# thetumbled/pulsar-tlaplus

Measured on AMD Instinct MI355X. Metric: distinct states/sec, compaction.tla scaled cfg, 1/2/4/8 MI355X vs host TLC, higher is better.
Workload: dtype u64

## Files before the change

include/tlcgpu.h:

```cpp
#ifndef TLCGPU_H
#define TLCGPU_H
#include <stdint.h>

#ifdef __cplusplus
extern "C" {
#endif

#define TLCG_ABI_VERSION 4
#define TLCG_MAX_SET 63
#define TLCG_MAX_INV 8

enum {
  TLCG_INV_TYPESAFE = 0,
  TLCG_INV_COMPACTED_LEDGER_LEAK = 1,
  TLCG_INV_HORIZON_CORRECTNESS = 2,
  TLCG_INV_DUP_NULLKEY_MESSAGE = 3,
  TLCG_INV_USER = 16
};

enum {
  TLCG_ACT_INIT = -1,
  TLCG_ACT_PRODUCER = 0,
  TLCG_ACT_PHASE_ONE,
  TLCG_ACT_PHASE_TWO_WRITE,
// ... 35 lines not shown
typedef struct tlcg_opts {
  int32_t device;
  int32_t log2_fpset_slots;
  uint64_t state_capacity;
  int32_t tlc_order;
  int32_t rank, world;
  int32_t partition;
  int32_t engine;
  int32_t spill;
  uint64_t device_store_cap;
  int32_t fpset_spill;
  int32_t log2_fpset_max;
  int32_t outdegree;
  int32_t reserved[1];
} tlcg_opts;

enum { TLCG_ENGINE_AUTO = 0, TLCG_ENGINE_GLOBAL = 1, TLCG_ENGINE_COMPONENT = 2,
       TLCG_ENGINE_TREE = 3  };

typedef struct tlcg_stats {
  uint64_t generated;
  uint64_t distinct;
  uint64_t frontier;
  int32_t depth;
  int32_t status;
  int32_t invariant;
  int32_t action;
  uint64_t event_gidx;
  double fp_collision_optimistic;
  double kernel_ms;
  double expand_ms;
  uint64_t levels_redone;
  uint64_t engine;
  uint64_t jit_used;
  uint64_t host_states;
  uint64_t fpset_host_states;
  uint64_t transport;
  uint64_t tlc_exact;
} tlcg_stats;

typedef struct tlcg_ctx tlcg_ctx;

int tlcg_abi_version(void);
int tlcg_check_model(const tlcg_model* m, char* err, int32_t cap);
int tlcg_state_bits(const tlcg_model* m);
int tlcg_state_words(const tlcg_model* m);
uint64_t tlcg_init_count(const tlcg_model* m);

int tlcg_create(const tlcg_model* m, const tlcg_opts* o, tlcg_ctx** out);
void tlcg_destroy(tlcg_ctx* c);
const char* tlcg_last_error(const tlcg_ctx* c);

int tlcg_init(tlcg_ctx* c, tlcg_stats* st);
int tlcg_step_level(tlcg_ctx* c, tlcg_stats* st);
int tlcg_run(tlcg_ctx* c, tlcg_stats* st);

int tlcg_level_sizes(tlcg_ctx* c, uint64_t* out, int32_t cap, int32_t* n);
int tlcg_trace(tlcg_ctx* c, uint64_t* states, int32_t* actions, int32_t cap, int32_t* len);
int tlcg_state_at(tlcg_ctx* c, uint64_t gidx, uint64_t* state, uint64_t* parent_ref);
int tlcg_copy_states(tlcg_ctx* c, uint64_t first, uint64_t n, uint64_t* out);
int tlcg_trace_words(tlcg_ctx* c, uint64_t* states, int32_t* actions, int32_t cap, int32_t* len);
int tlcg_state_at_words(tlcg_ctx* c, uint64_t gidx, uint64_t* state, uint64_t* parent_ref);
int tlcg_copy_states_words(tlcg_ctx* c, uint64_t first, uint64_t n, uint64_t* out);
int tlcg_tlc_stop_stats(tlcg_ctx* c, uint64_t* generated, uint64_t* distinct, uint64_t* left_on_queue);
int tlcg_outdegree(tlcg_ctx* c, uint64_t* hist, int32_t cap, int32_t* n);
int tlcg_expansions(tlcg_ctx* c, uint64_t* out);
int tlcg_level_generated(tlcg_ctx* c, uint64_t* out, int32_t cap, int32_t* n);
int tlcg_ordinal_bits(const tlcg_model* m);
int tlcg_action_of_ordinal(const tlcg_model* m, int32_t ordinal);

int tlcg_decode(const tlcg_model* m, uint64_t state, char* buf, int32_t cap);
uint64_t tlcg_host_init_state(const tlcg_model* m, uint64_t idx);
int tlcg_host_successors(const tlcg_model* m, uint64_t state, uint64_t* out, int32_t* actions, int32_t cap);
int tlcg_host_check_invariants(const tlcg_model* m, uint64_t state);
int tlcg_decode_words(const tlcg_model* m, const uint64_t* state, char* buf, int32_t cap);
int tlcg_host_init_state_words(const tlcg_model* m, uint64_t idx, uint64_t* out);
int tlcg_host_successors_words(const tlcg_model* m, const uint64_t* state, uint64_t* out, int32_t* actions,
                               int32_t cap);
int tlcg_host_check_invariants_words(const tlcg_model* m, const uint64_t* state);
int tlcg_host_check_invariants_batch(const tlcg_model* m, const uint64_t* states, uint64_t n, int32_t* out);
int64_t tlcg_host_component_selfcheck(const tlcg_model* m, uint64_t first, uint64_t n);
int64_t tlcg_host_lane_inv_selfcheck(const tlcg_model* m);
int64_t tlcg_host_lane_owner_selfcheck(const tlcg_model* m, int* overflow);
int64_t tlcg_host_lane_owner_word(const tlcg_model* m, uint32_t code);
int tlcg_host_tree_slot_probes(const tlcg_model* m, uint64_t comp, int64_t* out);
int64_t tlcg_host_termination_counterexample(const tlcg_model* m);
enum { TLCG_FAIR_NONE = 0, TLCG_FAIR_WF_NEXT = 1 };
enum { TLCG_LIVE_HOLDS = 0, TLCG_LIVE_STUTTERING = 1, TLCG_LIVE_CYCLE = 2 };
typedef struct tlcg_liveness {
  int32_t holds;
  int32_t kind;
  int32_t fairness;
  int32_t depth;
  uint64_t states_notp;
  uint64_t init_notp;
  uint64_t edges_notp;
  uint64_t stuck;
  uint64_t on_cycles;
  uint64_t peel_rounds;
  int32_t trace_len;
  int32_t loop_to;
  int32_t back_action;
  int32_t reserved;
  double kernel_ms;
  double wall_ms;
} tlcg_liveness;
int tlcg_check_termination(const tlcg_model* m, const tlcg_opts* o, int32_t fairness, tlcg_liveness* out,
                           uint64_t* states, int32_t* actions, int32_t cap, int32_t* len, char* err,
                           int32_t err_cap);
int tlcg_liveness_graph_selftest(const uint32_t* row, const uint32_t* col, const uint8_t* is_p, uint32_t n,
                                 uint32_t n_init, int32_t words, const tlcg_opts* o, int32_t fairness,
                                 tlcg_liveness* out, uint64_t* states, int32_t* actions, int32_t cap, int32_t* len,
                                 char* err, int32_t err_cap);

enum { TLCG_PROP_EVENTUALLY = 0, TLCG_PROP_INFINITELY_OFTEN = 1, TLCG_PROP_LEADS_TO = 2 };
typedef struct tlcg_property {
  tlcg_liveness lv;
  int32_t form;
  int32_t seed_at;
  uint64_t reachable;
  uint64_t seeds;
  int64_t error_state;
  double classify_ms;
} tlcg_property;
int tlcg_check_property(const tlcg_model* m, const tlcg_opts* o, int32_t fairness, const char* name,
                        tlcg_property* out, uint64_t* states, int32_t* actions, int32_t cap, int32_t* len,
                        char* err, int32_t err_cap);
int tlcg_property_graph_selftest(const uint32_t* row, const uint32_t* col, const uint8_t* is_p, const uint8_t* is_q,
                                 uint32_t n, uint32_t n_init, int32_t words, const tlcg_opts* o, int32_t fairness,
                                 int32_t form, tlcg_property* out, uint64_t* states, int32_t* actions, int32_t cap,
                                 int32_t* len, char* err, int32_t err_cap);
int tlcg_host_property_form(const tlcg_model* m, const char* name, int32_t* form, char* err, int32_t cap);
int tlcg_host_property_eval(const tlcg_model* m, const char* name, const uint64_t* states, uint64_t n, uint8_t* out);

typedef struct tlcg_action_property {
  int32_t holds;
  int32_t depth;
  uint64_t reachable;
  uint64_t steps;
  uint64_t violating;
  uint64_t erroring;
  int32_t step_depth;
  int32_t step_action;
  int32_t trace_len;
  int32_t reserved;
  int64_t error_state;
  double kernel_ms;
  double check_ms;
  double wall_ms;
} tlcg_action_property;
int tlcg_check_action_property(const tlcg_model* m, const tlcg_opts* o, const char* name, tlcg_action_property* out,
                               uint64_t* states, int32_t* actions, int32_t cap, int32_t* len, char* err,
                               int32_t err_cap);
int tlcg_action_property_graph_selftest(const uint32_t* row, const uint32_t* col, const uint8_t* verdict, uint32_t n,
                                        uint32_t n_init, int32_t words, const tlcg_opts* o,
                                        tlcg_action_property* out, uint64_t* states, int32_t* actions, int32_t cap,
                                        int32_t* len, char* err, int32_t err_cap);
int tlcg_host_action_property_form(const tlcg_model* m, const char* name, uint32_t* var_mask, char* err, int32_t cap);
int tlcg_host_action_property_eval(const tlcg_model* m, const char* name, const uint64_t* pairs, uint64_t n,
                                   uint8_t* out);
int tlcg_action_eval_selftest(const tlcg_model* m, const tlcg_opts* o, const char* name, const uint64_t* pairs,
                              uint64_t n, uint8_t* out, char* err, int32_t cap);

int tlcg_peer_access(int32_t n);
int tlcg_device_count(void);
int tlcg_owner(tlcg_ctx* c, uint64_t state);
// ... 44 lines not shown
```

pulsar-tlaplus_amd/csrc/component_lane.h:

```cpp
#pragma once
#if !defined(__HIPCC_RTC__)
#include "component_body.h"
#endif

namespace tlcg {

#ifndef TLCG_LANE_R
#define TLCG_LANE_R 16
#endif
constexpr int LANE_R = TLCG_LANE_R;
#ifndef TLCG_LANE_STEP_TAB
#define TLCG_LANE_STEP_TAB 1
#endif
#ifndef TLCG_LANE_INV_FEAT
#define TLCG_LANE_INV_FEAT 1
#endif
#if defined(TLCG_USER_INV) || defined(TLCG_LANE_INV_UNCOND)
#undef TLCG_LANE_INV_FEAT
#define TLCG_LANE_INV_FEAT 0
#endif
#ifndef TLCG_LANE_OWNER_RING
#define TLCG_LANE_OWNER_RING 1
#endif
#if !TLCG_LANE_STEP_TAB
#undef TLCG_LANE_OWNER_RING
#define TLCG_LANE_OWNER_RING 0
#endif
#ifndef TLCG_LANE_FP_REG
#define TLCG_LANE_FP_REG 1
#endif
#ifndef TLCG_LANE_LEVEL_LDS
#define TLCG_LANE_LEVEL_LDS 1
#endif
#ifndef TLCG_LANE_CRASH_SKIP
#define TLCG_LANE_CRASH_SKIP 1
#endif

template <bool B>
struct lane_with2 {
  static constexpr bool value = B;
};

__device__ __forceinline__ uint32_t lane_wave_sum(uint32_t x) {
  x += (uint32_t)__builtin_amdgcn_update_dpp(0, (int)x, 0x111, 0xf, 0xf, true);
  x += (uint32_t)__builtin_amdgcn_update_dpp(0, (int)x, 0x112, 0xf, 0xf, true);
  x += (uint32_t)__builtin_amdgcn_update_dpp(0, (int)x, 0x114, 0xf, 0xf, true);
  x += (uint32_t)__builtin_amdgcn_update_dpp(0, (int)x, 0x118, 0xf, 0xf, true);
  return (uint32_t)__builtin_amdgcn_readlane((int)x, 15) + (uint32_t)__builtin_amdgcn_readlane((int)x, 31) +
         (uint32_t)__builtin_amdgcn_readlane((int)x, 47) + (uint32_t)__builtin_amdgcn_readlane((int)x, 63);
}

template <int K, bool OD = false>
__device__ __forceinline__ void component_lane_body(const CompArgs& a, const Layout& L) {
  static_assert(K <= 64, "records and the 16-bit level sums take K <= 64");
  static_assert(64 * (K - 2) * 4 < 65536, "level_add's 16-bit halves");
  constexpr int T = LANE_T, NW = T / 32, R = LANE_R;
  constexpr int LV = TLCG_CODE_MAXLV < COMP_MAXLV ? TLCG_CODE_MAXLV : COMP_MAXLV;
#if TLCG_LANE_OWNER_RING
  typedef uint32_t ring_t;
#else
  typedef uint16_t ring_t;
#endif
  __shared__ ring_t ring[R][64];
#if TLCG_LANE_FP_REG
  __shared__ u64 owner[T];
#else
  __shared__ uint32_t bits[NW][64];
  __shared__ uint32_t owner[T];
#endif
  constexpr int LVS = LV + (OD ? 3 : 0);
  static_assert(LVS <= 64 && (K - 2) * 4 + 1 < 256, "one lane per level sum; OD packs three counts above lgen's 8 bits");
  __shared__ unsigned long long lvl_sh[LVS];
#if TLCG_LANE_STEP_TAB
  __shared__ u64 steps[STEP_TAB];
#endif
  const int lane = threadIdx.x;
  const int mb = L.msg_sh + L.N * L.mw;
  const uint32_t mult = a.lane_mult;
#if TLCG_LANE_FP_REG
  for (int i = lane; i < T; i += 64) owner[i] = (u64)a.lane_owner[2 * i] | ((u64)a.lane_owner[2 * i + 1] << 32);
#else
  for (int i = lane; i < T; i += 64) owner[i] = a.lane_owner[2 * i];
#endif
#if TLCG_LANE_STEP_TAB
  for (int i = lane; i < STEP_TAB; i += 64) steps[i] = compactor_step_entry(L, i);
#endif
  if (lane < LVS) lvl_sh[lane] = 0;
  uint32_t gen = 0, dist = 0, nexp = 0;
  __syncthreads();
  auto level_add = [&](bool add, int lvc, uint32_t x) {
#if TLCG_LANE_LEVEL_LDS
    if (add) atomicAdd(&lvl_sh[lvc], (unsigned long long)(x & 0xFFFFu) | ((unsigned long long)(x >> 16) << 32));
#else
    const unsigned long long m = __ballot(add);
    if (!m) return;
    const int l0 = __builtin_amdgcn_readlane(lvc, __ffsll((long long)m) - 1);
    if (!__ballot(add && lvc != l0)) {
      const uint32_t s = lane_wave_sum(add ? x : 0u);
      if (lane == 0) atomicAdd(&lvl_sh[l0], (unsigned long long)(s & 0xFFFFu) | ((unsigned long long)(s >> 16) << 32));
    } else if (add) {
      atomicAdd(&lvl_sh[lvc], (unsigned long long)(x & 0xFFFFu) | ((unsigned long long)(x >> 16) << 32));
    }
#endif
  };
  for (u64 b = blockIdx.x; b * 64 < a.n_comp; b += gridDim.x) {
    const u64 ci = b * 64 + (u64)lane;
    const bool act = ci < a.n_comp;
    const u64 entry = act ? (a.list ? a.list[ci] : a.comp0 + ci) : 0;
    const u64 idx0 = entry & ((1ull << 40) - 1);
    const int counted = (int)(entry >> 40);
#if TLCG_LANE_FP_REG
    u64 fp = 0;
#else
#pragma unroll
    for (int i = 0; i < NW; ++i) bits[i][lane] = 0u;
#endif
    const u64 s0 = init_state(L, idx0);
    CodeConsts ccon = code_consts(L, comp_msgs_init(L, s0));
#ifdef TLCG_USER_INV
    code_consts_user(L, ccon);
#endif
#if TLCG_LANE_INV_FEAT
    const uint32_t cmask = lane_inv_mask(L, ccon);
#endif
#if TLCG_LANE_STEP_TAB
    const int term_c = lane_term_consts(L, ccon);
#endif
    const __amdgpu_buffer_rsrc_t rsrc = __builtin_amdgcn_make_buffer_rsrc(
        reinterpret_cast<uint32_t*>(a.store) + b * (u64)K * 64, (short)0, K * 64 * 4, 0x00020000);
    constexpr int OOB = 0x7fffffff;
    const unsigned loff = (unsigned)lane * 4u;
    int head = 0, tail = 0, level = 0, lvl_start = 0, lvl_end = 0;
    bool alive = act, ovf = false, stop = false;
    uint32_t lgen = 0, lvgen = 0;
    u64 lev = NO_EVENT;
    const lkey k0 = act ? (lkey)(s0 >> mb) : 0;
    const ckey c0 = code_encode(L, k0);
    const unsigned p0 = lane_slot(c0, mult);
    const uint32_t ow0 = (uint32_t)owner[p0];
    if (act && (code_decode(L, ccon, c0) != k0 || (ow0 & 0xFFFFu) != c0 + 1u)) {
      ovf = true;
      alive = false;
    }
    if (alive) {
#if TLCG_LANE_FP_REG
      fp = 1ull << (uint32_t)(owner[p0] >> 32);
#else
      bits[p0 >> 5][lane] = 1u << (p0 & 31);
#endif
#if TLCG_LANE_OWNER_RING
      ring[0][lane] = ow0;
#else
      ring[0][lane] = (uint16_t)c0;
#endif
      tail = 1;
      __builtin_amdgcn_raw_buffer_store_b32(comp_record(c0, 0, 0), rsrc, (int)loff, 0, 0);
      lgen = 1;
      const int c = check_invariants_direct(L, ccon, c0);
      if (c >= 0) {
        lev = make_comp_event(0, idx0, 0, 0, (c & 1) ? EVK_INV_ERROR : EVK_VIOLATION, c >> 1);
        alive = false;
        stop = true;
      }
    }
    lvl_end = tail;
#if TLCG_LANE_OWNER_RING
    uint32_t cur = ow0;
#else
    ckey cur = c0;
#endif
    while (__ballot(alive)) {
      const int tail0 = tail;
#if TLCG_LANE_OWNER_RING
      const ckey s = (cur & 0xFFFFu) - 1u;
      uint32_t nxt = 0, first_new = 0;
#else
      const ckey s = cur;
      ckey nxt = 0, first_new = 0;
#endif
      bool out = false, rare = false, dl = false, u1 = false, u2 = false;
      int q1 = INV_UNKNOWN + 1, q2 = INV_UNKNOWN + 1;
      ckey t = 0;
      int action = 0;
#if TLCG_LANE_OWNER_RING
      nxt = ring[(head + 1) & (R - 1)][lane];
      const uint32_t six = (cur >> LANE_OWNER_STEP_SH) & (uint32_t)(STEP_TAB - 1);
      uint32_t term = 0;
      const int r = compactor_step_ent(L, ccon, steps[six], six & 7u, s, &t, &action, &term);
#else
      nxt = ring[(head + 1) & (R - 1)][lane];
#if TLCG_LANE_STEP_TAB
      uint32_t term = 0;
      const int r = compactor_step_tab(L, ccon, steps, s, &t, &action, &term);
#else
      const int r = compactor_step_cb(L, ccon, s, &t, &action);
#endif
#endif
      auto expand = [&](auto with2) __attribute__((always_inline)) {
        constexpr bool W2 = decltype(with2)::value;
        ckey t2 = 0;
        bool crash = false;
        if constexpr (W2) crash = crash_step_c(L, s, &t2) != 0;
        const unsigned p1 = lane_slot(t, mult), p2 = W2 ? lane_slot(t2, mult) : 0u;
#if TLCG_LANE_FP_REG
        const u64 oe1 = owner[p1], oe2 = W2 ? owner[p2] : 0ull;
        const uint32_t o1 = (uint32_t)oe1, o2 = (uint32_t)oe2;
#else
        const uint32_t o1 = owner[p1], o2 = W2 ? owner[p2] : 0u;
        const uint32_t w1 = bits[p1 >> 5][lane];
        uint32_t w2 = W2 ? bits[p2 >> 5][lane] : 0u;
#endif
#ifndef TLCG_LANE_NO_SCHED_BARRIER
        __builtin_amdgcn_sched_barrier(0);
#endif
        const bool e1 = alive && r == 1, e2 = W2 && alive && crash;
        const bool in1 = (o1 & 0xFFFFu) == t + 1u, in2 = W2 && (o2 & 0xFFFFu) == t2 + 1u;
        out = (e1 && !in1) || (e2 && !in2);
        bool new2 = false;
#if TLCG_LANE_FP_REG
        const u64 b1 = 1ull << (uint32_t)(oe1 >> 32);
        const bool new1 = e1 && in1 && !(fp & b1) && !out;
        fp |= new1 ? b1 : 0ull;
        if constexpr (W2) {
          const u64 b2 = 1ull << (uint32_t)(oe2 >> 32);
          new2 = e2 && in2 && !(fp & b2) && !out;
          fp |= new2 ? b2 : 0ull;
        }
#else
        const uint32_t b1 = 1u << (p1 & 31);
        const bool new1 = e1 && in1 && !(w1 & b1) && !out;
        bits[p1 >> 5][lane] = new1 ? w1 | b1 : w1;
        if constexpr (W2) {
          const uint32_t b2 = 1u << (p2 & 31);
          if ((p2 >> 5) == (p1 >> 5) && new1) w2 |= b1;
          new2 = e2 && in2 && !(w2 & b2) && !out;
          bits[p2 >> 5][lane] = new2 ? w2 | b2 : w2;
        }
#endif
#if TLCG_LANE_OWNER_RING
        ring[tail & (R - 1)][lane] = o1;
        if constexpr (W2) ring[(tail + (new1 ? 1 : 0)) & (R - 1)][lane] = o2;
#else
        ring[tail & (R - 1)][lane] = (uint16_t)t;
        if constexpr (W2) ring[(tail + (new1 ? 1 : 0)) & (R - 1)][lane] = (uint16_t)t2;
#endif
#ifndef TLCG_NO_STORE
        __builtin_amdgcn_raw_buffer_store_b32(comp_record(t, head, action), rsrc,
                                              new1 ? (int)((unsigned)tail * 256u + loff) : OOB, 0, 0);
        if constexpr (W2)
          __builtin_amdgcn_raw_buffer_store_b32(comp_record(t2, head, ACT_CRASH), rsrc,
                                                new2 ? (int)((unsigned)(tail + (new1 ? 1 : 0)) * 256u + loff) : OOB,
                                                0, 0);
#endif
#if TLCG_LANE_OWNER_RING
        first_new = W2 ? (new1 ? o1 : o2) : o1;
#else
        first_new = W2 ? (new1 ? t : t2) : t;
#endif
        tail += (new1 ? 1 : 0) + (new2 ? 1 : 0);
#if TLCG_LANE_STEP_TAB
        const int nsucc = (e1 ? 1 : 0) + (e2 ? 1 : 0) + (alive ? selfloop_count_tab(L, term_c, term) : 0);
#else
        const int nsucc = (e1 ? 1 : 0) + (e2 ? 1 : 0) + (alive ? selfloop_count_c(L, ccon, s) : 0);
#endif
        lvgen += (unsigned)nsucc;
        if constexpr (OD) lgen += alive ? 256u << (8 * (tail - tail0)) : 0u;
#if TLCG_LANE_INV_FEAT && !defined(TLCG_NO_INV)
        u1 = new1 && ((o1 >> 16) & cmask);
        if constexpr (W2) u2 = new2 && ((o2 >> 16) & cmask);
#elif !defined(TLCG_NO_INV)
#ifdef TLCG_LANE_INV_UNCOND
        q1 = check_invariants_cbt(L, ccon, t) + 1;
        if constexpr (W2) q2 = check_invariants_cbt(L, ccon, t2) + 1;
#else
        q1 = new1 ? check_invariants_cbt(L, ccon, t) + 1 : 0;
        if constexpr (W2) q2 = new2 ? check_invariants_cbt(L, ccon, t2) + 1 : 0;
#endif
        u1 = new1 && q1 != 0;
        if constexpr (W2) u2 = new2 && q2 != 0;
#endif
        dl = nsucc == 0 && L.check_deadlock;
        rare = alive && ((r == 2) | dl | u1 | u2);
      };
#if TLCG_LANE_CRASH_SKIP
      if (__ballot(alive && crash_enabled_c(L, s))) expand(lane_with2<true>{});
      else expand(lane_with2<false>{});
#else
      expand(lane_with2<true>{});
#endif
      if (__ballot(rare)) {
        if (rare) {
          int ev1 = u1 ? q1 : 0, ev2 = u2 ? q2 : 0;
          ckey t2 = 0;
          if (u2) crash_step_c(L, s, &t2);
#pragma nounroll
          for (int i = 0; i < 2; ++i) {
            if ((i ? ev2 : ev1) == INV_UNKNOWN + 1) {
              const int e = check_invariants_direct(L, ccon, i ? t2 : t) + 1;
              if (i) ev2 = e;
              else ev1 = e;
            }
          }
          u64 k = r == 2 ? make_comp_event(level + 1, idx0, head, action, EVK_ACTION_ERROR, action)
                  : dl ? make_comp_event(level + 1, idx0, head, 15, EVK_DEADLOCK, 0)
                                                   : NO_EVENT;
          if (ev1) k = min(k, make_comp_event(level + 1, idx0, head, action, ((ev1 - 1) & 1) ? EVK_INV_ERROR : EVK_VIOLATION, (ev1 - 1) >> 1));
          if (ev2) k = min(k, make_comp_event(level + 1, idx0, head, ACT_CRASH, ((ev2 - 1) & 1) ? EVK_INV_ERROR : EVK_VIOLATION, (ev2 - 1) >> 1));
          lev = min(lev, k);
          stop = stop || k != NO_EVENT;
        }
      }
      if (alive) ++head;
      cur = head < tail0 ? nxt : first_new;
      bool brk = alive && head >= tail;
      const bool ended = alive && head == lvl_end;
      if (__ballot(ended)) {
        const int lvc = level < LV ? level : LV - 1;
        level_add(ended && level >= counted, lvc, (uint32_t)(lvl_end - lvl_start) | (lvgen << 16));
        if (ended) {
          lgen += lvgen;
          lvgen = 0;
          ++level;
          lvl_start = head;
          lvl_end = tail;
          const bool deep = level >= LV;
          ovf = ovf || deep;
          brk = brk || deep || stop;
        }
      }
      const bool full = alive && !brk && (tail > K - 2 || tail - head > R - 2);
      ovf = ovf || full || out;
      alive = alive && !(brk || full || out);
    }
    if (act && ovf) {
      const unsigned long long k = atomicAdd(a.ovf_n, 1ull);
      a.ovf_list[k] = idx0 | ((u64)(level > counted ? level : counted) << 40);
    }
    const bool fin = act && !ovf;
    const int lvc = level < LV ? level : LV - 1;
    level_add(fin && tail > lvl_start && level >= counted, lvc, (uint32_t)(tail - lvl_start));
    if constexpr (OD) {
#pragma unroll
      for (int i = 0; i < 3; ++i) {
        const u64 w = wave_sum_u64(fin ? (lgen >> (8 + 8 * i)) & 0xFFu : 0u);
        if (lane == 0 && w) atomicAdd(&lvl_sh[LV + i], (unsigned long long)w);
      }
    }
    if (fin) {
      gen += OD ? lgen & 0xFFu : lgen;
      dist += (uint32_t)tail;
      nexp += (uint32_t)head;
    }
    if (__ballot(fin && lev != NO_EVENT)) {
      unsigned long long ev = fin ? (unsigned long long)lev : NO_EVENT;
#pragma unroll
      for (int off = 32; off > 0; off >>= 1) ev = min(ev, (unsigned long long)__shfl_xor(ev, off));
      if (lane == 0) atomicMin(a.event, ev);
    }
  }
  const u64 g64 = wave_sum_u64(gen), d64 = wave_sum_u64(dist), x64 = wave_sum_u64(nexp);
  __syncthreads();
  const u64 so = a.nstripe > 1 ? (u64)(blockIdx.x % (unsigned)a.nstripe) * a.stripe : 0;
  if (lane == 0) {
    if (x64 && a.expansions) atomicAdd(&a.expansions[so], (unsigned long long)x64);
    if (g64) atomicAdd(&a.totals[so + 0], (unsigned long long)g64);
    if (d64) atomicAdd(&a.totals[so + 1], (unsigned long long)d64);
  }
  if constexpr (OD)
    if (lane < 3 && lvl_sh[LV + lane]) atomicAdd(&a.outdeg[so + lane], lvl_sh[LV + lane]);
  if (lane < LV && lvl_sh[lane]) {
    atomicAdd(&a.lvl[so + lane], lvl_sh[lane] & 0xffffffffull);
    if (lvl_sh[lane] >> 32) atomicAdd(&a.lvl_gen[so + lane], lvl_sh[lane] >> 32);
  }
}

}
```

pulsar-tlaplus_amd/csrc/host_model.cpp:

```cpp
#include "host_model.h"

#include "component_code.h"
#include "component_model.h"

#include <algorithm>
#include <cstdio>
#include <cstring>
#include <sstream>
#include <unordered_set>

namespace tlcg {

static const char* kPhaseName[6] = {
    "Compactor_In_PhaseOne", "Compactor_In_PhaseTwoWrite", "Compactor_In_PhaseTwoUpdateContext",
    "Compactor_In_PhaseTwoUpdateHorizon", "Compactor_In_PhaseTwoPersistCusror",
    "Compactor_In_PhaseTwoDeleteLedger"};

bool build_model(const tlcg_model& m, HostModel* out, std::string* err) {
  auto fail = [&](const std::string& s) {
    if (err) *err = s;
    return false;
  };
  if (m.msg_sent_limit < 0) return fail("Assumption MessageSentLimit \\in Nat is false.");
  if (m.compaction_times_limit < 0) return fail("Assumption CompactionTimesLimit \\in Nat is false.");
// ... 903 lines not shown
  int64_t checked = 0;
  for (int len = 0; len <= L.N; ++len)
    for (int f = 0; f < 32; ++f) {
      CodeConsts kc{};
      kc.len = (uint32_t)len;
      kc.ledbits = 1u;
      kc.msgs_ok = f & 1;
      kc.hz_live = (f >> 1) & 1;
      kc.hz_false = (f >> 2) & 1;
      kc.dn0 = (f >> 3) & 1;
      kc.dn1 = (f >> 4) & 1;
      const uint32_t imask = lane_inv_mask(L, kc);
      const int term_c = lane_term_consts(L, kc);
      for (ckey cd = 0; cd < (1u << code_bits(L)); ++cd) {
        ckey t = 0;
        int act = -1;
        uint32_t term = 0;
        compactor_step_tab(L, kc, tab, cd, &t, &act, &term);
        if (((lane_inv_feat(L, cd) & imask) != 0) != (check_invariants_cb(L, kc, cd) != -1) ||
            selfloop_count_tab(L, term_c, term) != selfloop_count_c(L, kc, cd))
          return -(1 + checked);
        ++checked;
      }
    }
  return checked;
}

int64_t tlcg_host_lane_owner_selfcheck(const tlcg_model* m, int* overflow) {
  HostModel hm;
  std::string e;
  if (overflow) *overflow = 0;
  if (!m || !build_model(*m, &hm, &e)) return -1;
  const Layout& L = hm.L;
  std::vector<uint32_t> owner(2 * LANE_T);
  uint32_t mult = 0;
  const bool taken = build_lane_phash(hm, &mult, owner.data(), nullptr);
  if (L.producer || code_bits(L) > 16) return taken ? -1 : 0;
  const u128 s0 = init_state<u128>(L, 0);
  const CodeConsts kc = code_consts(L, comp_msgs_init(L, (u64)s0));
  std::vector<uint32_t> q{code_encode_w<u128>(L, s0)};
  std::unordered_set<uint32_t> seen{q[0]};
  for (size_t head = 0; head < q.size() && q.size() <= 64; ++head) {
    ckey t = 0, t2 = 0;
    int act = 0;
    if (compactor_step_cb(L, kc, q[head], &t, &act) == 1 && seen.insert(t).second) q.push_back(t);
    if (crash_step_c(L, q[head], &t2) && seen.insert(t2).second) q.push_back(t2);
  }
  auto plain_index = [&](uint32_t c) {
    uint32_t mx = 0;
    for (int j = 0; j < L.C; ++j)
      if ((c >> j) & 1u) mx = (uint32_t)j + 1u;
    return ((c >> (L.C + 2)) & 7u) | (((c >> L.C) & 1u) << 3) | (mx << 4);
  };
  bool ovf = q.size() > 62;
  for (uint32_t c : q)
    if (c + 1u >= (1u << 16) || lane_inv_feat(L, c) >= (1u << 9) || plain_index(c) >= (1u << 6)) ovf = true;
  if (overflow) *overflow = ovf ? 1 : 0;
  if (!taken) return 0;
  if (ovf) return -1;
  u64 tab[STEP_TAB];
  for (int i = 0; i < STEP_TAB; ++i) tab[i] = compactor_step_entry(L, i);
  std::vector<int> slot_used(LANE_T, 0);
  u64 dense_seen = 0;
  for (size_t i = 0; i < q.size(); ++i) {
    const ckey c = q[i];
    const unsigned sl = lane_slot(c, mult);
    const uint32_t w = owner[2 * sl], d = owner[2 * sl + 1];
    const uint32_t ix = w >> LANE_OWNER_STEP_SH;
    ckey t = 0, t3 = 0;
    int a1 = -1, a3 = -1;
    const int r1 = compactor_step_cb(L, kc, c, &t, &a1);
    const int r3 = ix < (uint32_t)STEP_TAB ? compactor_step_ent(L, kc, tab[ix], ix & 7u, c, &t3, &a3) : -1;
    if (slot_used[sl]++ || (w & 0xFFFFu) != c + 1u || ((w >> LANE_OWNER_FEAT_SH) & 0x1FFu) != lane_inv_feat(L, c) ||
        ix != plain_index(c) || r3 != r1 || (r1 == 1 && t3 != t) || (r1 && a3 != a1) || d != (uint32_t)i || d >= q.size() || ((dense_seen >> d) & 1))
      return -(1 + (int64_t)i);
    dense_seen |= 1ull << d;
  }
  if (dense_seen != (q.size() >= 64 ? ~0ull : (1ull << q.size()) - 1)) return -(1 + (int64_t)q.size());
  for (int s = 0; s < LANE_T; ++s)
    if (!slot_used[s] && (owner[2 * s] || owner[2 * s + 1])) return -(1 + (int64_t)q.size());
  return (int64_t)q.size();
}

int64_t tlcg_host_lane_owner_word(const tlcg_model* m, uint32_t code) {
  HostModel hm;
  std::string e;
  if (!m || !build_model(*m, &hm, &e)) return -1;
  return (int64_t)lane_owner_word(hm.L, code);
}

}
```

pulsar-tlaplus_amd/python/tlcgpu.py:

```python
from __future__ import annotations

import ctypes as C
import os
from dataclasses import dataclass, field
from typing import List, Optional, Sequence, Tuple

HERE = os.path.dirname(os.path.abspath(__file__))
LIB_PATH = os.environ.get("TLCG_LIB") or os.path.normpath(os.path.join(HERE, "..", "lib", "libtlcgpu.so"))

MAX_SET = 63
MAX_INV = 8

INVARIANTS = ("TypeSafe", "CompactedLedgerLeak", "CompactionHorizonCorrectness", "DuplicateNullKeyMessage")
INV_USER = 16
ACTIONS = ("Producer", "CompactorPhaseOne", "CompactorPhaseTwoWrite", "CompactorPhaseTwoUpdateContext",
           "CompactorPhaseTwoUpdateHorizon", "CompactorPhaseTwoPersistCusror", "CompactorPhaseTwoDeleteLedger",
           "BrokerCrash", "Consumer", "Terminating")
STATUS = {0: "running", 1: "ok", 2: "invariant", 3: "deadlock", 4: "action_error", 5: "invariant_error"}
ENGINES = {"auto": 0, "global": 1, "component": 2, "tree": 3}
ENGINE_NAMES = {1: "global", 2: "component", 3: "tree"}


class tlcg_model(C.Structure):
    _fields_ = [("msg_sent_limit", C.c_int32), ("compaction_times_limit", C.c_int32),
# ... 9 lines not shown
class tlcg_opts(C.Structure):
    _fields_ = [("device", C.c_int32), ("log2_fpset_slots", C.c_int32), ("state_capacity", C.c_uint64),
                ("tlc_order", C.c_int32), ("rank", C.c_int32), ("world", C.c_int32), ("partition", C.c_int32),
                ("engine", C.c_int32), ("spill", C.c_int32), ("device_store_cap", C.c_uint64),
                ("fpset_spill", C.c_int32), ("log2_fpset_max", C.c_int32), ("outdegree", C.c_int32),
                ("reserved", C.c_int32 * 1)]


class tlcg_stats(C.Structure):
    _fields_ = [("generated", C.c_uint64), ("distinct", C.c_uint64), ("frontier", C.c_uint64),
                ("depth", C.c_int32), ("status", C.c_int32), ("invariant", C.c_int32), ("action", C.c_int32),
                ("event_gidx", C.c_uint64), ("fp_collision_optimistic", C.c_double), ("kernel_ms", C.c_double),
                ("expand_ms", C.c_double), ("levels_redone", C.c_uint64), ("engine", C.c_uint64),
                ("jit_used", C.c_uint64), ("host_states", C.c_uint64), ("fpset_host_states", C.c_uint64),
                ("transport", C.c_uint64), ("tlc_exact", C.c_uint64)]


class tlcg_liveness(C.Structure):
    _fields_ = [("holds", C.c_int32), ("kind", C.c_int32), ("fairness", C.c_int32), ("depth", C.c_int32),
                ("states_notp", C.c_uint64), ("init_notp", C.c_uint64), ("edges_notp", C.c_uint64),
                ("stuck", C.c_uint64), ("on_cycles", C.c_uint64), ("peel_rounds", C.c_uint64),
                ("trace_len", C.c_int32), ("loop_to", C.c_int32), ("back_action", C.c_int32),
                ("reserved", C.c_int32), ("kernel_ms", C.c_double), ("wall_ms", C.c_double)]


class tlcg_property(C.Structure):
    _fields_ = [("lv", tlcg_liveness), ("form", C.c_int32), ("seed_at", C.c_int32), ("reachable", C.c_uint64),
                ("seeds", C.c_uint64), ("error_state", C.c_int64), ("classify_ms", C.c_double)]


class tlcg_action_property(C.Structure):
    _fields_ = [("holds", C.c_int32), ("depth", C.c_int32), ("reachable", C.c_uint64), ("steps", C.c_uint64),
                ("violating", C.c_uint64), ("erroring", C.c_uint64), ("step_depth", C.c_int32),
                ("step_action", C.c_int32), ("trace_len", C.c_int32), ("reserved", C.c_int32),
                ("error_state", C.c_int64), ("kernel_ms", C.c_double), ("check_ms", C.c_double),
                ("wall_ms", C.c_double)]


VARIABLES = ("messages", "compactedLedgers", "cursor", "compactorState", "phaseOneResult", "compactionHorizon",
             "compactedTopicContext", "crashTimes", "consumeTimes")
FAIRNESS = {"none": 0, "wf": 1}
PROP_FORMS = {0: "eventually", 1: "infinitely_often", 2: "leads_to"}
PROP_FORM_IDS = {v: k for k, v in PROP_FORMS.items()}
LIVE_KINDS = {0: "holds", 1: "stuttering", 2: "cycle"}

_lib = None


def load_library(path: str = LIB_PATH):
    global _lib
    if _lib is not None:
        return _lib
    if not os.path.exists(path):
        raise RuntimeError(f"libtlcgpu.so not built at {path}: run __graft_entry__.build()")
    lib = C.CDLL(path)
    P, U64, I32 = C.c_void_p, C.c_uint64, C.c_int32
    M, O, S = C.POINTER(tlcg_model), C.POINTER(tlcg_opts), C.POINTER(tlcg_stats)
    sig = {
        "tlcg_abi_version": (C.c_int, []),
        "tlcg_check_model": (C.c_int, [M, C.c_char_p, I32]),
        "tlcg_state_bits": (C.c_int, [M]),
        "tlcg_init_count": (U64, [M]),
        "tlcg_create": (C.c_int, [M, O, C.POINTER(P)]),
        "tlcg_destroy": (None, [P]),
        "tlcg_last_error": (C.c_char_p, [P]),
        "tlcg_init": (C.c_int, [P, S]),
        "tlcg_step_level": (C.c_int, [P, S]),
        "tlcg_run": (C.c_int, [P, S]),
        "tlcg_level_sizes": (C.c_int, [P, C.POINTER(U64), I32, C.POINTER(I32)]),
        "tlcg_level_generated": (C.c_int, [P, C.POINTER(U64), I32, C.POINTER(I32)]),
        "tlcg_trace": (C.c_int, [P, C.POINTER(U64), C.POINTER(I32), I32, C.POINTER(I32)]),
        "tlcg_state_at": (C.c_int, [P, U64, C.POINTER(U64), C.POINTER(U64)]),
        "tlcg_copy_states": (C.c_int, [P, U64, U64, C.POINTER(U64)]),
        "tlcg_ordinal_bits": (C.c_int, [M]),
        "tlcg_action_of_ordinal": (C.c_int, [M, I32]),
        "tlcg_decode": (C.c_int, [M, U64, C.c_char_p, I32]),
        "tlcg_host_init_state": (U64, [M, U64]),
        "tlcg_host_successors": (C.c_int, [M, U64, C.POINTER(U64), C.POINTER(I32), I32]),
        "tlcg_host_check_invariants": (C.c_int, [M, U64]),
        "tlcg_host_component_selfcheck": (C.c_int64, [M, U64, U64]),
        "tlcg_host_lane_inv_selfcheck": (C.c_int64, [M]),
        "tlcg_host_lane_owner_selfcheck": (C.c_int64, [M, C.POINTER(C.c_int)]),
        "tlcg_host_lane_owner_word": (C.c_int64, [M, C.c_uint32]),
        "tlcg_host_tree_slot_probes": (C.c_int, [M, U64, C.POINTER(C.c_int64)]),
        "tlcg_host_termination_counterexample": (C.c_int64, [M]),
        "tlcg_owner": (C.c_int, [P, U64]),
        "tlcg_expand": (C.c_int, [P, S]),
        "tlcg_outbox": (C.c_int, [P, I32, C.POINTER(P), C.POINTER(U64)]),
        "tlcg_inbox": (C.c_int, [P, U64, C.POINTER(P)]),
        "tlcg_absorb": (C.c_int, [P, U64, S]),
        "tlcg_end_level": (C.c_int, [P, S]),
        "tlcg_outbox_read": (C.c_int, [P, I32, P, U64]),
        "tlcg_outbox_gather": (C.c_int, [P, P]),
        "tlcg_state_words": (C.c_int, [M]),
        "tlcg_checkpoint": (C.c_int, [P, C.c_char_p]),
        "tlcg_recover": (C.c_int, [P, C.c_char_p, S]),
        "tlcg_decode_words": (C.c_int, [M, C.POINTER(U64), C.c_char_p, I32]),
        "tlcg_host_init_state_words": (C.c_int, [M, U64, C.POINTER(U64)]),
        "tlcg_host_successors_words": (C.c_int, [M, C.POINTER(U64), C.POINTER(U64), C.POINTER(I32), I32]),
        "tlcg_host_check_invariants_words": (C.c_int, [M, C.POINTER(U64)]),
        "tlcg_host_check_invariants_batch": (C.c_int, [M, C.POINTER(U64), U64, C.POINTER(I32)]),
        "tlcg_trace_words": (C.c_int, [P, C.POINTER(U64), C.POINTER(I32), I32, C.POINTER(I32)]),
        "tlcg_state_at_words": (C.c_int, [P, U64, C.POINTER(U64), C.POINTER(U64)]),
        "tlcg_copy_states_words": (C.c_int, [P, U64, U64, C.POINTER(U64)]),
        "tlcg_tlc_stop_stats": (C.c_int, [P, C.POINTER(U64), C.POINTER(U64), C.POINTER(U64)]),
        "tlcg_outdegree": (C.c_int, [P, C.POINTER(U64), I32, C.POINTER(I32)]),
        "tlcg_expansions": (C.c_int, [P, C.POINTER(U64)]),
        "tlcg_absorb_records": (C.c_int, [P, P, U64, S]),
        "tlcg_stream": (P, [P]),
        "tlcg_peer_access": (C.c_int, [I32]),
        "tlcg_device_count": (C.c_int, []),
        "tlcg_exchange_local": (C.c_int, [C.POINTER(P), I32, C.POINTER(U64)]),
        "tlcg_partition_closed": (C.c_int, [P]),
        "tlcg_run_node": (C.c_int, [M, O, I32, S, C.POINTER(U64), I32, C.POINTER(I32), C.c_char_p, I32]),
        "tlcg_run_node_trace": (C.c_int, [M, O, I32, S, C.POINTER(U64), I32, C.POINTER(I32), C.POINTER(U64),
                                          C.POINTER(I32), I32, C.POINTER(I32), C.c_char_p, I32]),
        "tlcg_node_create": (C.c_int, [M, O, I32, C.POINTER(P), C.c_char_p, I32]),
        "tlcg_node_run": (C.c_int, [P, S, C.POINTER(U64), I32, C.POINTER(I32), C.POINTER(U64), C.POINTER(I32), I32,
                                    C.POINTER(I32), C.c_char_p, I32]),
        "tlcg_node_destroy": (None, [P]),
        "tlcg_comm_available": (C.c_int, []),
        "tlcg_comm_unique_id": (C.c_int, [P, I32]),
        "tlcg_comm_init": (C.c_int, [P, P, I32]),
        "tlcg_comm_size": (C.c_int, [P]),
        "tlcg_run_comm": (C.c_int, [P, S, C.POINTER(U64), I32, C.POINTER(I32)]),
        "tlcg_check_termination": (C.c_int, [M, O, I32, C.POINTER(tlcg_liveness), C.POINTER(U64),
                                             C.POINTER(I32), I32, C.POINTER(I32), C.c_char_p, I32]),
        "tlcg_liveness_graph_selftest": (C.c_int, [C.POINTER(C.c_uint32), C.POINTER(C.c_uint32),
                                                   C.POINTER(C.c_uint8), C.c_uint32, C.c_uint32, I32, O, I32,
                                                   C.POINTER(tlcg_liveness), C.POINTER(U64), C.POINTER(I32), I32,
                                                   C.POINTER(I32), C.c_char_p, I32]),
        "tlcg_check_property": (C.c_int, [M, O, I32, C.c_char_p, C.POINTER(tlcg_property), C.POINTER(U64),
                                          C.POINTER(I32), I32, C.POINTER(I32), C.c_char_p, I32]),
        "tlcg_property_graph_selftest": (C.c_int, [C.POINTER(C.c_uint32), C.POINTER(C.c_uint32),
                                                   C.POINTER(C.c_uint8), C.POINTER(C.c_uint8), C.c_uint32,
                                                   C.c_uint32, I32, O, I32, I32, C.POINTER(tlcg_property),
                                                   C.POINTER(U64), C.POINTER(I32), I32, C.POINTER(I32), C.c_char_p,
                                                   I32]),
        "tlcg_host_property_form": (C.c_int, [M, C.c_char_p, C.POINTER(I32), C.c_char_p, I32]),
        "tlcg_host_property_eval": (C.c_int, [M, C.c_char_p, C.POINTER(U64), U64, C.POINTER(C.c_uint8)]),
        "tlcg_check_action_property": (C.c_int, [M, O, C.c_char_p, C.POINTER(tlcg_action_property), C.POINTER(U64),
                                                 C.POINTER(I32), I32, C.POINTER(I32), C.c_char_p, I32]),
        "tlcg_action_property_graph_selftest": (C.c_int, [C.POINTER(C.c_uint32), C.POINTER(C.c_uint32),
                                                          C.POINTER(C.c_uint8), C.c_uint32, C.c_uint32, I32, O,
                                                          C.POINTER(tlcg_action_property), C.POINTER(U64),
                                                          C.POINTER(I32), I32, C.POINTER(I32), C.c_char_p, I32]),
        "tlcg_host_action_property_form": (C.c_int, [M, C.c_char_p, C.POINTER(C.c_uint32), C.c_char_p, I32]),
        "tlcg_host_action_property_eval": (C.c_int, [M, C.c_char_p, C.POINTER(U64), U64, C.POINTER(C.c_uint8)]),
        "tlcg_action_eval_selftest": (C.c_int, [M, O, C.c_char_p, C.POINTER(U64), U64, C.POINTER(C.c_uint8),
                                                C.c_char_p, I32]),
        "tlcg_jit_selftest": (C.c_int, [M, C.c_char_p, I32, C.c_char_p, I32][:1] + [C.c_char_p, C.c_char_p, I32]),
        "tlcg_user_eval_selftest": (C.c_int, [M, O, C.POINTER(U64), U64, I32, C.POINTER(C.c_uint8), C.c_char_p, I32]),
    }
    for name, (res, args) in sig.items():
        fn = getattr(lib, name)
        fn.restype = res
        fn.argtypes = args
    _lib = lib
    return lib


@dataclass
class Model:
    msg_sent_limit: int = 3
    compaction_times_limit: int = 3
    consume_times_limit: int = 2
# ... 63 lines not shown
                "-producer", str(int(self.model_producer)), "-consumer", str(int(self.model_consumer)),
                "-inv", ",".join(self.invariants)] + ([] if self.check_deadlock else ["-nodeadlock"])


def check_model(model: Model) -> Optional[str]:
    lib = load_library()
    buf = C.create_string_buffer(512)
    m = model.to_c()
    return None if lib.tlcg_check_model(C.byref(m), buf, 512) == 0 else buf.value.decode()


def state_bits(model: Model) -> int:
    m = model.to_c()
    return load_library().tlcg_state_bits(C.byref(m))


def init_count(model: Model) -> int:
    m = model.to_c()
    return load_library().tlcg_init_count(C.byref(m))


def state_words(model: Model) -> int:
    m = model.to_c()
    return load_library().tlcg_state_words(C.byref(m))


def _to_words(state: int, w: int):
    return (C.c_uint64 * w)(*[(state >> (64 * i)) & 0xFFFFFFFFFFFFFFFF for i in range(w)])


def _from_words(buf, i: int, w: int) -> int:
    return sum(int(buf[i * w + k]) << (64 * k) for k in range(w))


def decode(model: Model, state: int) -> str:
    lib = load_library()
    m = model.to_c()
    buf = C.create_string_buffer(1 << 16)
    n = lib.tlcg_decode_words(C.byref(m), _to_words(state, state_words(model)), buf, len(buf))
    if n < 0:
        raise ValueError("bad model")
    return buf.value.decode()


def host_init_state(model: Model, idx: int) -> int:
    m = model.to_c()
    w = state_words(model)
    out = (C.c_uint64 * 2)()
    if load_library().tlcg_host_init_state_words(C.byref(m), idx, out) != 0:
        raise ValueError("bad model")
    return _from_words(out, 0, w)


def host_successors(model: Model, state: int) -> List[Tuple[str, int]]:
    lib = load_library()
    m = model.to_c()
    w = state_words(model)
    cap = 8192
    out = (C.c_uint64 * (cap * w))()
    acts = (C.c_int32 * cap)()
    n = lib.tlcg_host_successors_words(C.byref(m), _to_words(state, w), out, acts, cap)
    if n < 0:
        raise RuntimeError("evaluation error")
    return [(ACTIONS[acts[i]], _from_words(out, i, w)) for i in range(n)]


def host_component_selfcheck(model: Model, first: int, n: int) -> int:
    m = model.to_c()
    return load_library().tlcg_host_component_selfcheck(C.byref(m), C.c_uint64(first), C.c_uint64(n))


def host_lane_inv_selfcheck(model: Model) -> int:
    m = model.to_c()
    return load_library().tlcg_host_lane_inv_selfcheck(C.byref(m))


def host_lane_owner_selfcheck(model: Model):
    m = model.to_c()
    ovf = C.c_int(0)
    n = load_library().tlcg_host_lane_owner_selfcheck(C.byref(m), C.byref(ovf))
    return n, bool(ovf.value)


def host_lane_owner_word(model: Model, code: int) -> int:
    m = model.to_c()
    return load_library().tlcg_host_lane_owner_word(C.byref(m), C.c_uint32(code))


def host_tree_slot_probes(model: Model, comp: int):
    m = model.to_c()
    out = (C.c_int64 * 3)()
    r = load_library().tlcg_host_tree_slot_probes(C.byref(m), C.c_uint64(comp), out)
    if r == -2:
        raise ValueError("bad model")
    return None if r < 0 else (out[0], out[1], out[2])


def host_check_invariants_batch(model: Model, states: Sequence[int]) -> List[int]:
    m = model.to_c()
    w = state_words(model)
    buf = (C.c_uint64 * (len(states) * w))()
    for i, s in enumerate(states):
        for k in range(w):
            buf[i * w + k] = (s >> (64 * k)) & 0xFFFFFFFFFFFFFFFF
    out = (C.c_int32 * max(1, len(states)))()
    if load_library().tlcg_host_check_invariants_batch(C.byref(m), buf, len(states), out) != 0:
        raise ValueError(check_model(model) or "bad model")
    return list(out)[:len(states)]


USER_EVAL_PATHS = {"interpreter": 0, "word": 1, "code": 2, "tables": 3}


def user_eval_states(model: Model, states: Sequence[int], path: str, device: int = 0) -> List[bytes]:
    lib = load_library()
    m = model.to_c()
    o = tlcg_opts()
    o.device = device
    w = state_words(model)
    users = model.user_names()
    nu = len(dict.fromkeys(n for n in model.invariants if n in users))
    n = len(states)
    buf = (C.c_uint64 * max(1, n * w))()
    for i, s in enumerate(states):
        for k in range(w):
            buf[i * w + k] = (s >> (64 * k)) & 0xFFFFFFFFFFFFFFFF
    out = (C.c_uint8 * max(1, n * nu))()
    err = C.create_string_buffer(4096)
    rc = lib.tlcg_user_eval_selftest(C.byref(m), C.byref(o), buf, n, USER_EVAL_PATHS[path], out, err, len(err))
    if rc != 0:
        raise RuntimeError(f"tlcg_user_eval_selftest: {rc}: {err.value.decode()}")
    raw = bytes(out)[:n * nu]
    return [raw[k::nu] for k in range(nu)]


def host_check_invariants(model: Model, state: int) -> int:
    m = model.to_c()
    return load_library().tlcg_host_check_invariants_words(C.byref(m), _to_words(state, state_words(model)))


@dataclass
class Liveness:
    holds: bool
    kind: str
    fairness: str
    depth: int
    states_notp: int
    init_notp: int
    edges_notp: int
    stuck: int
    on_cycles: int
    peel_rounds: int
    trace: List[Tuple[str, int]] = field(default_factory=list)
    loop_to: int = -1
    back_action: Optional[str] = None
    kernel_ms: float = 0.0
    wall_ms: float = 0.0


def check_termination(model: Model, fairness: str = "none", device: int = 0, state_capacity: int = 0,
                      log2_fpset_slots: int = 0) -> Liveness:
    lib = load_library()
    m = model.to_c()
    o = tlcg_opts()
    o.device, o.state_capacity, o.log2_fpset_slots = device, state_capacity, log2_fpset_slots
    out = tlcg_liveness()
# ... 496 lines not shown
```

Baseline: 434.4 billion.

## Replace per-lane BFS ring with shared dense-index table assuming canonical discovery order

When the perfect-hash owner table records each code's dense BFS index, the lane kernel stops keeping a per-lane ring of queued states and a visited-bit fingerprint. It instead checks that each newly discovered successor's precomputed index equals the current tail, and reads the next state to expand from a shared byidx table. Any out-of-order discovery is treated as an overflow and falls back to the slow path. This removes the LDS ring writes and reads and the fingerprint updates per expansion, at the cost of depending on every component sharing the same BFS order. A host self-check is added to verify that assumption.

```diff
diff --git a/include/tlcgpu.h b/include/tlcgpu.h
--- a/include/tlcgpu.h
+++ b/include/tlcgpu.h
@@ -141,6 +141,7 @@
 int64_t tlcg_host_component_selfcheck(const tlcg_model* m, uint64_t first, uint64_t n);
 int64_t tlcg_host_lane_inv_selfcheck(const tlcg_model* m);
 int64_t tlcg_host_lane_owner_selfcheck(const tlcg_model* m, int* overflow);
+int64_t tlcg_host_lane_prefix_selfcheck(const tlcg_model* m, uint64_t first, uint64_t n);
 int64_t tlcg_host_lane_owner_word(const tlcg_model* m, uint32_t code);
 int tlcg_host_tree_slot_probes(const tlcg_model* m, uint64_t comp, int64_t* out);
 int64_t tlcg_host_termination_counterexample(const tlcg_model* m);
diff --git a/pulsar-tlaplus_amd/csrc/component_lane.h b/pulsar-tlaplus_amd/csrc/component_lane.h
--- a/pulsar-tlaplus_amd/csrc/component_lane.h
+++ b/pulsar-tlaplus_amd/csrc/component_lane.h
@@ -34,6 +34,13 @@
 #endif
 #ifndef TLCG_LANE_CRASH_SKIP
 #define TLCG_LANE_CRASH_SKIP 1
+#endif
+#ifndef TLCG_LANE_PREFIX
+#define TLCG_LANE_PREFIX 1
+#endif
+#if !TLCG_LANE_FP_REG || !TLCG_LANE_OWNER_RING
+#undef TLCG_LANE_PREFIX
+#define TLCG_LANE_PREFIX 0
 #endif
 
 template <bool B>
@@ -61,7 +68,12 @@
 #else
   typedef uint16_t ring_t;
 #endif
+#if TLCG_LANE_PREFIX
+  __shared__ uint32_t byidx[64];
+  (void)R;
+#else
   __shared__ ring_t ring[R][64];
+#endif
 #if TLCG_LANE_FP_REG
   __shared__ u64 owner[T];
 #else
@@ -87,6 +99,14 @@
 #endif
   if (lane < LVS) lvl_sh[lane] = 0;
   uint32_t gen = 0, dist = 0, nexp = 0;
+#if TLCG_LANE_PREFIX
+  byidx[lane] = 0u;
+  __syncthreads();
+  for (int i = lane; i < T; i += 64) {
+    const uint32_t w = a.lane_owner[2 * i], d = a.lane_owner[2 * i + 1];
+    if (w && d < 64u) byidx[d] = w;
+  }
+#endif
   __syncthreads();
   auto level_add = [&](bool add, int lvc, uint32_t x) {
 #if TLCG_LANE_LEVEL_LDS
@@ -109,7 +129,8 @@
     const u64 entry = act ? (a.list ? a.list[ci] : a.comp0 + ci) : 0;
     const u64 idx0 = entry & ((1ull << 40) - 1);
     const int counted = (int)(entry >> 40);
-#if TLCG_LANE_FP_REG
+#if TLCG_LANE_PREFIX
+#elif TLCG_LANE_FP_REG
     u64 fp = 0;
 #else
 #pragma unroll
@@ -138,17 +159,24 @@
     const ckey c0 = code_encode(L, k0);
     const unsigned p0 = lane_slot(c0, mult);
     const uint32_t ow0 = (uint32_t)owner[p0];
-    if (act && (code_decode(L, ccon, c0) != k0 || (ow0 & 0xFFFFu) != c0 + 1u)) {
+#if TLCG_LANE_PREFIX
+    const bool root_ok = (ow0 & 0xFFFFu) == c0 + 1u && (uint32_t)(owner[p0] >> 32) == 0u;
+#else
+    const bool root_ok = (ow0 & 0xFFFFu) == c0 + 1u;
+#endif
+    if (act && (code_decode(L, ccon, c0) != k0 || !root_ok)) {
       ovf = true;
       alive = false;
     }
     if (alive) {
-#if TLCG_LANE_FP_REG
+#if TLCG_LANE_PREFIX
+#elif TLCG_LANE_FP_REG
       fp = 1ull << (uint32_t)(owner[p0] >> 32);
 #else
       bits[p0 >> 5][lane] = 1u << (p0 & 31);
 #endif
-#if TLCG_LANE_OWNER_RING
+#if TLCG_LANE_PREFIX
+#elif TLCG_LANE_OWNER_RING
       ring[0][lane] = ow0;
 #else
       ring[0][lane] = (uint16_t)c0;
@@ -173,7 +201,11 @@
       const int tail0 = tail;
 #if TLCG_LANE_OWNER_RING
       const ckey s = (cur & 0xFFFFu) - 1u;
+#if TLCG_LANE_PREFIX
+      uint32_t nxt = 0;
+#else
       uint32_t nxt = 0, first_new = 0;
+#endif
 #else
       const ckey s = cur;
       ckey nxt = 0, first_new = 0;
@@ -183,7 +215,11 @@
       ckey t = 0;
       int action = 0;
 #if TLCG_LANE_OWNER_RING
+#if TLCG_LANE_PREFIX
+      nxt = byidx[(head + 1) & 63];
+#else
       nxt = ring[(head + 1) & (R - 1)][lane];
+#endif
       const uint32_t six = (cur >> LANE_OWNER_STEP_SH) & (uint32_t)(STEP_TAB - 1);
       uint32_t term = 0;
       const int r = compactor_step_ent(L, ccon, steps[six], six & 7u, s, &t, &action, &term);
@@ -217,7 +253,26 @@
         const bool in1 = (o1 & 0xFFFFu) == t + 1u, in2 = W2 && (o2 & 0xFFFFu) == t2 + 1u;
         out = (e1 && !in1) || (e2 && !in2);
         bool new2 = false;
-#if TLCG_LANE_FP_REG
+#if TLCG_LANE_PREFIX
+        const uint32_t d1 = (uint32_t)(oe1 >> 32), ut = (uint32_t)tail;
+        const bool n1 = e1 && in1 && d1 >= ut;
+        bool bad = n1 && d1 != ut;
+#ifdef TLCG_LANE_PREFIX_BREAK
+        bad = bad || (n1 && tail == (TLCG_LANE_PREFIX_BREAK));
+#endif
+        bool n2 = false;
+        if constexpr (W2) {
+          const uint32_t d2 = (uint32_t)(oe2 >> 32), ut2 = ut + (n1 ? 1u : 0u);
+          n2 = e2 && in2 && d2 >= ut2;
+          bad = bad || (n2 && d2 != ut2);
+#ifdef TLCG_LANE_PREFIX_BREAK
+          bad = bad || (n2 && (int)ut2 == (TLCG_LANE_PREFIX_BREAK));
+#endif
+        }
+        out = out || bad;
+        const bool new1 = n1 && !out;
+        new2 = n2 && !out;
+#elif TLCG_LANE_FP_REG
         const u64 b1 = 1ull << (uint32_t)(oe1 >> 32);
         const bool new1 = e1 && in1 && !(fp & b1) && !out;
         fp |= new1 ? b1 : 0ull;
@@ -237,7 +292,8 @@
           bits[p2 >> 5][lane] = new2 ? w2 | b2 : w2;
         }
 #endif
-#if TLCG_LANE_OWNER_RING
+#if TLCG_LANE_PREFIX
+#elif TLCG_LANE_OWNER_RING
         ring[tail & (R - 1)][lane] = o1;
         if constexpr (W2) ring[(tail + (new1 ? 1 : 0)) & (R - 1)][lane] = o2;
 #else
@@ -252,7 +308,8 @@
                                                 new2 ? (int)((unsigned)(tail + (new1 ? 1 : 0)) * 256u + loff) : OOB,
                                                 0, 0);
 #endif
-#if TLCG_LANE_OWNER_RING
+#if TLCG_LANE_PREFIX
+#elif TLCG_LANE_OWNER_RING
         first_new = W2 ? (new1 ? o1 : o2) : o1;
 #else
         first_new = W2 ? (new1 ? t : t2) : t;
@@ -311,7 +368,11 @@
         }
       }
       if (alive) ++head;
+#if TLCG_LANE_PREFIX
+      cur = nxt;
+#else
       cur = head < tail0 ? nxt : first_new;
+#endif
       bool brk = alive && head >= tail;
       const bool ended = alive && head == lvl_end;
       if (__ballot(ended)) {
@@ -328,7 +389,11 @@
           brk = brk || deep || stop;
         }
       }
+#if TLCG_LANE_PREFIX
+      const bool full = K < 64 && alive && !brk && tail > K - 2;
+#else
       const bool full = alive && !brk && (tail > K - 2 || tail - head > R - 2);
+#endif
       ovf = ovf || full || out;
       alive = alive && !(brk || full || out);
     }
diff --git a/pulsar-tlaplus_amd/csrc/host_model.cpp b/pulsar-tlaplus_amd/csrc/host_model.cpp
--- a/pulsar-tlaplus_amd/csrc/host_model.cpp
+++ b/pulsar-tlaplus_amd/csrc/host_model.cpp
@@ -1009,6 +1009,41 @@
   return (int64_t)q.size();
 }
 
+int64_t tlcg_host_lane_prefix_selfcheck(const tlcg_model* m, uint64_t first, uint64_t n) {
+  HostModel hm;
+  std::string e;
+  if (!m || !build_model(*m, &hm, &e)) return -1;
+  const Layout& L = hm.L;
+  std::vector<uint32_t> owner(2 * LANE_T);
+  uint32_t mult = 0;
+  if (!build_lane_phash(hm, &mult, owner.data(), nullptr)) return 0;
+  auto dense = [&](ckey c) -> int64_t {
+    const unsigned sl = lane_slot(c, mult);
+    return (owner[2 * sl] & 0xFFFFu) == c + 1u ? (int64_t)owner[2 * sl + 1] : -1;
+  };
+  int64_t kept = 0;
+  for (u64 idx = first; idx < first + n && idx < hm.n_init; ++idx) {
+    const u128 s0 = init_state<u128>(L, idx);
+    const CodeConsts kc = code_consts(L, comp_msgs_init(L, (u64)s0));
+    std::vector<ckey> q{code_encode_w<u128>(L, s0)};
+    std::unordered_set<uint32_t> seen{q[0]};
+    bool ok = dense(q[0]) == 0;
+    auto put = [&](ckey t) {
+      if (!seen.insert(t).second) return;
+      ok = ok && dense(t) == (int64_t)q.size();
+      q.push_back(t);
+    };
+    for (size_t head = 0; ok && head < q.size(); ++head) {
+      ckey t = 0, t2 = 0;
+      int act = 0;
+      if (compactor_step_cb(L, kc, q[head], &t, &act) == 1) put(t);
+      if (ok && crash_step_c(L, q[head], &t2)) put(t2);
+    }
+    kept += ok ? 1 : 0;
+  }
+  return kept;
+}
+
 int64_t tlcg_host_lane_owner_word(const tlcg_model* m, uint32_t code) {
   HostModel hm;
   std::string e;
diff --git a/pulsar-tlaplus_amd/python/tlcgpu.py b/pulsar-tlaplus_amd/python/tlcgpu.py
--- a/pulsar-tlaplus_amd/python/tlcgpu.py
+++ b/pulsar-tlaplus_amd/python/tlcgpu.py
@@ -115,6 +115,7 @@
         "tlcg_host_lane_inv_selfcheck": (C.c_int64, [M]),
         "tlcg_host_lane_owner_selfcheck": (C.c_int64, [M, C.POINTER(C.c_int)]),
         "tlcg_host_lane_owner_word": (C.c_int64, [M, C.c_uint32]),
+        "tlcg_host_lane_prefix_selfcheck": (C.c_int64, [M, U64, U64]),
         "tlcg_host_tree_slot_probes": (C.c_int, [M, U64, C.POINTER(C.c_int64)]),
         "tlcg_host_termination_counterexample": (C.c_int64, [M]),
         "tlcg_owner": (C.c_int, [P, U64]),
@@ -344,6 +345,11 @@
     return n, bool(ovf.value)
 
 
+def host_lane_prefix_selfcheck(model: Model, first: int, n: int) -> int:
+    m = model.to_c()
+    return load_library().tlcg_host_lane_prefix_selfcheck(C.byref(m), C.c_uint64(first), C.c_uint64(n))
+
+
 def host_lane_owner_word(model: Model, code: int) -> int:
     m = model.to_c()
     return load_library().tlcg_host_lane_owner_word(C.byref(m), C.c_uint32(code))
```

Measured after the change: 511.2 billion, median of 6. 1.18x the previous value.
